# hsinnan75/MapCaller

Hardware: AMD Instinct MI355X
Metric: reads/sec (150 bp PE vs GRCh38) at 1/2/4/8 MI355X; SAM CIGAR bit-exact (higher is better)
Workload: dtype u64/int32; 1 GPU; synthetic GRCh38-sized genome, 3100 Mbp (synthetic: GRCh38 is unavailable offline; repeat landscape in the detail record), 4000000 pairs x 150 bp PE per step per GPU (sub 0.005, ins 0.001, del 0.001 per base), -alg ksw2

## Files before the change

mapcaller_amd/csrc/mcx_pack.h:

```cpp
#ifndef MCX_PACK_H
#define MCX_PACK_H
#include "mcx_fm.h"

namespace mcx {

static inline MCX_HD uint32_t pack_alignbyte(uint32_t hi, uint32_t lo, unsigned b)
{
#if defined(__HIP_DEVICE_COMPILE__)
    return __builtin_amdgcn_alignbyte(hi, lo, b);
#else
    return (uint32_t)((((uint64_t)hi << 32) | lo) >> (8 * (b & 3)));
#endif
}

static inline MCX_HD U4 load16_span(const U4 *base16, uint64_t A, int n)
{
    const U4 *q = base16 + (A >> 4);
    const U4 lo = q[0];
    const unsigned sh = (unsigned)(A & 15);
    if (sh == 0) return lo;
    U4 hi; hi.x = hi.y = hi.z = hi.w = 0;
    if ((int)sh + n > 16) hi = q[1];
    const unsigned qd = sh >> 2, b = sh & 3;
    uint32_t s0, s1, s2, s3, s4;
    switch (qd) {
    case 0: s0 = lo.x; s1 = lo.y; s2 = lo.z; s3 = lo.w; s4 = hi.x; break;
    case 1: s0 = lo.y; s1 = lo.z; s2 = lo.w; s3 = hi.x; s4 = hi.y; break;
    case 2: s0 = lo.z; s1 = lo.w; s2 = hi.x; s3 = hi.y; s4 = hi.z; break;
    default: s0 = lo.w; s1 = hi.x; s2 = hi.y; s3 = hi.z; s4 = hi.w; break;
    }
    U4 r;
    r.x = pack_alignbyte(s1, s0, b); r.y = pack_alignbyte(s2, s1, b);
    r.z = pack_alignbyte(s3, s2, b); r.w = pack_alignbyte(s4, s3, b);
    return r;
}

static inline MCX_HD void pack4(uint32_t w, bool comp, uint32_t &codes, uint32_t &flags, uint32_t &lower)
{
    const uint32_t c = w & 0xDFDFDFDFu;
#define MCX_ZERO_BYTES(t) (~((((t) & 0x7F7F7F7Fu) + 0x7F7F7F7Fu) | (t) | 0x7F7F7F7Fu))
    const uint32_t member = (MCX_ZERO_BYTES(c ^ 0x41414141u) | MCX_ZERO_BYTES(c ^ 0x43434343u) | MCX_ZERO_BYTES(c ^ 0x47474747u) | MCX_ZERO_BYTES(c ^ 0x54545454u)) >> 7;
#undef MCX_ZERO_BYTES
    const uint32_t h = (c >> 1) & 0x03030303u;
    uint32_t code = h ^ ((h >> 1) & 0x01010101u);
    if (comp) code ^= 0x03030303u;
    code &= member * 3u;
    const uint32_t y = __builtin_bswap32(code), n = __builtin_bswap32(member ^ 0x01010101u);
    codes = (y | (y >> 6) | (y >> 12) | (y >> 18)) & 0xFFu;
    flags = (n | (n >> 7) | (n >> 14) | (n >> 21)) & 0xFu;
    const uint32_t l = __builtin_bswap32((w >> 5) & 0x01010101u);
    lower = (l | (l >> 7) | (l >> 14) | (l >> 21)) & 0xFu;
}

static inline MCX_HD void pack16_span(const U4 *base16, uint64_t A0, int rlen, int flipped, int i0, uint32_t &codes, uint32_t &flags, uint32_t &odd)
{
    int n = rlen - i0; if (n > 16) n = 16;
    codes = 0; flags = 0xFFFFu; odd = 0;
    if (n <= 0) return;
    const int a0 = flipped ? rlen - i0 - n : i0;
    U4 v = load16_span(base16, A0 + (uint64_t)a0, n);
    if (flipped) {
        const U4 t = v;
        v.x = __builtin_bswap32(t.w); v.y = __builtin_bswap32(t.z); v.z = __builtin_bswap32(t.y); v.w = __builtin_bswap32(t.x);
    }
    uint32_t c0, f0, c1, f1, c2, f2, c3, f3, l0, l1, l2, l3;
    pack4(v.x, flipped != 0, c0, f0, l0); pack4(v.y, flipped != 0, c1, f1, l1); pack4(v.z, flipped != 0, c2, f2, l2); pack4(v.w, flipped != 0, c3, f3, l3);
    uint32_t c = (c0 << 24) | (c1 << 16) | (c2 << 8) | c3, f = (f0 << 12) | (f1 << 8) | (f2 << 4) | f3, o = f | (l0 << 12) | (l1 << 8) | (l2 << 4) | l3;
    if (n < 16) {
        const int pad = 16 - n;
        if (flipped) { c <<= 2 * pad; f = (f << pad) & 0xFFFFu; o = (o << pad) & 0xFFFFu; }
        else { c &= ~0u << (2 * pad); o &= ~0u << pad; }
        f |= (1u << pad) - 1u;
        if (!flipped) f &= 0xFFFFu;
    }
    codes = c; flags = f; odd = o & 0xFFFFu;
}

static inline MCX_HD void pack_row_ends(int rlen, uint32_t *row)
{
    const int nc = (rlen + 15) >> 4, nmw = (rlen + 31) >> 5;
    row[nc] = 0u;
    row[nc + 1 + nmw] = 0xFFFFFFFFu;
}

static inline MCX_HD void pack_unit32(const U4 *base16, uint64_t A0, int rlen, int flipped, int m, uint32_t *row, uint32_t &has_n, uint32_t &odd)
{
    const int nc = (rlen + 15) >> 4;
    uint32_t c0, f0, c1, f1, o0, o1;
    pack16_span(base16, A0, rlen, flipped, 32 * m, c0, f0, o0);
    pack16_span(base16, A0, rlen, flipped, 32 * m + 16, c1, f1, o1);
    row[2 * m] = c0;
    if (2 * m + 1 < nc) row[2 * m + 1] = c1;
    row[nc + 1 + m] = (f0 << 16) | f1;
    const int left = rlen - 32 * m;
    has_n = ((f0 << 16) | f1) & (left >= 32 ? ~0u : ~(0xFFFFFFFFu >> left));
    odd = o0 | o1;
}

}
#endif
```

mapcaller_amd/csrc/mcx_pipeline.hip:

```cpp
#include "mcx_ctx.h"
#include "mcx_pack.h"
#include <hipcub/hipcub.hpp>

static thread_local std::string g_err;
static int fail(int code, const std::string &msg) { g_err = msg; return code; }
int mcx_set_error(int code, const std::string &msg) { return fail(code, msg); }
extern "C" const char *mcx_last_error(void) { return g_err.c_str(); }
extern "C" int mcx_device_count(void)
{
    int n = 0;
    if (hipGetDeviceCount(&n) != hipSuccess) return 0;
    return n;
}

struct EndsLds { int64_t pos[kLdsEnds]; int32_t chr[kLdsEnds]; };

static __device__ __forceinline__ void stage_ends(IndexView &ix, EndsLds &l)
{
    if (ix.n_ends <= kLdsEnds) {
        for (int i = threadIdx.x; i < ix.n_ends; i += blockDim.x) { l.pos[i] = ix.end_pos[i]; l.chr[i] = ix.end_chr[i]; }
        __syncthreads();
        ix.end_pos = l.pos; ix.end_chr = l.chr;
    }
}

static __device__ __forceinline__ void make_reads(const Ctx &cx, const ReadBatch &rb, uint32_t pair, ReadRef rd[2])
{
    const int nr = cx.pm.paired ? 2 : 1;
    for (int s = 0; s < nr; s++) {
        uint32_t r = pair * nr + s;
        rd[s].ascii = rb.bases + rb.off[r];
        rd[s].rlen = (int32_t)(rb.off[r + 1] - rb.off[r]);
        rd[s].flipped = (cx.pm.paired && s == 1) ? 1 : 0;
        rd[s].codes = (cx.packed && !(cx.read_ext[r] >> 31)) ? cx.packed + (uint64_t)r * cx.wpad : nullptr;
#ifdef MCX_DEBUG_NO_CODES
        rd[s].codes = nullptr;
#endif
    }
}

struct SeedOut {
    uint2 *tasks;
    uint32_t *n_tasks;
    uint32_t task_cap;
    uint32_t *read_ext;
    uint32_t *read_blocks;
    const uint32_t *packed;
    int wpad;
    uint32_t *queue;
    const uint8_t *src_state; Layout src_lay; Caps src_caps;
};

static __device__ __forceinline__ void pack_read_part(const ReadBatch &rb, uint32_t r, int m, int paired, int wpad, uint32_t *out, uint32_t *any_n, uint8_t *odd_flag)
{
    const uint32_t a = rb.off[r];
    const int rlen = (int)(rb.off[r + 1] - a), flipped = (paired && (r & 1)) ? 1 : 0, nmw = (rlen + 31) >> 5;
    if (packed_words(rlen) > wpad) return;
    uint32_t *o = out + (uint64_t)r * wpad;
    const uint8_t *p = rb.bases + a;
    const uint32_t sh = (uint32_t)((uintptr_t)p & 15);
    if (m < nmw) {
        uint32_t has_n, odd;
        pack_unit32((const U4 *)(p - sh), (uint64_t)sh, rlen, flipped, m, o, has_n, odd);
        if (odd_flag && odd) atomicOr((uint32_t *)(odd_flag + (r & ~3u)), 2u << (8 * (r & 3)));
        if (has_n) atomicOr(any_n, 1u);
    } else if (m == nmw) pack_row_ends(rlen, o);
}

__global__ void __launch_bounds__(256) k_pack_reads(ReadBatch rb, int paired, int wpad, int tpr, uint32_t *out, uint32_t *any_n, uint8_t *odd_flag)
{
    const uint64_t t = (uint64_t)blockIdx.x * blockDim.x + threadIdx.x;
    const uint32_t r = (uint32_t)(t / (uint32_t)tpr);
    if (r < rb.n_reads) pack_read_part(rb, r, (int)(t % (uint32_t)tpr), paired, wpad, out, any_n, odd_flag);
}

void pack_reads(const ReadBatch &rb, int paired, int wpad, int tpr, uint32_t *out, uint32_t *any_n, uint8_t *odd_flag, hipStream_t s)
{
    k_pack_reads<<<(unsigned)(((uint64_t)rb.n_reads * (uint64_t)tpr + 255) / 256), 256, 0, s>>>(rb, paired, wpad, tpr, out, any_n, odd_flag);
}

constexpr int kSeedReadsPerLane = 4;


static inline int seed_reads_per_lane(uint64_t n_reads) { return n_reads >= (uint64_t)1 << 21 ? kSeedReadsPerLane : (n_reads >= (uint64_t)1 << 19 ? 2 : 1); }

#ifndef MCX_SEED_WAVES
#define MCX_SEED_WAVES 1
#endif
#ifdef MCX_SEED_STATS
__device__ unsigned long long g_seed_hist[2][24];
#endif
__global__ void __launch_bounds__(256, MCX_SEED_WAVES) k_seed(Ctx cx, ReadBatch rb, PairSel sel, SeedOut so, int pk_words, int reads_per_lane, int fm_budget)
{
    extern __shared__ uint32_t pk_lds[];
    const int nr = cx.pm.paired ? 2 : 1;
    const uint32_t total = sel.n * nr;
    const int lane = threadIdx.x & 63;
    const uint64_t lt_mask = lane == 0 ? 0ull : (~0ull >> (64 - lane));
    const uint32_t chunk = 64u * (uint32_t)reads_per_lane;
    PackedRead pk; pk.w = pk_lds + threadIdx.x; pk.stride = blockDim.x; pk.n_code = 0;
    bool have = false;
    uint32_t lr = 0, r = 0, nm = 0;
    int rlen = 0, p = 0, n = 0;
    int64_t ext = 0, blocks = 0;
    Hit *hits = nullptr;
    uint32_t has_n = 0;
    int cap = cx.caps.hit_seed;
    auto finish_read = [&]() {
        so.read_ext[r] = (uint32_t)ext | (has_n << 31); so.read_blocks[r] = (uint32_t)blocks | ((uint32_t)n << 20);
#ifdef MCX_SEED_STATS
        { const int bk = blocks ? 64 - __clzll((unsigned long long)blocks) : 0; atomicAdd(&g_seed_hist[0][bk], 1ull); atomicAdd(&g_seed_hist[1][bk], (unsigned long long)blocks); }
#endif
        if (cx.ix.sa_full) return;
        const int keep = n <= cx.caps.hit_seed ? n : 0;
        int todo = 0;
        for (int i = 0; i < keep; i++) if (!(hits[i].len & kHitResolved)) todo++;
        uint32_t at = todo ? atomicAdd(so.n_tasks, (uint32_t)todo) : 0u;
        for (int i = 0; i < keep; i++) {
            if (hits[i].len & kHitResolved) { hits[i].len &= ~kHitResolved; continue; }
            if (at < so.task_cap) so.tasks[at] = make_uint2(lr, (uint32_t)i);
            at++;
        }
    };
    SeedWalk walk; walk.phase = 0;
    uint32_t q_next = 0, q_end = 0;
    bool dry = false;
    for (;;) {
        const uint64_t need = __ballot(!have);
        bool fresh = false;
        if (need && !dry) {
            const uint32_t rank = (uint32_t)__popcll(need & lt_mask), want = (uint32_t)__popcll(need);
            uint32_t given = 0;
            while (given < want) {
                if (q_next == q_end) {
                    uint32_t b = 0;
                    if (lane == 0) b = atomicAdd(so.queue, chunk);
                    b = __shfl(b, 0, 64);
                    if (b >= total) { dry = true; break; }
                    q_next = b; q_end = min(b + chunk, total);
                }
                const uint32_t take = min(want - given, q_end - q_next);
                if (!have && !fresh && rank >= given && rank < given + take) { lr = q_next + (rank - given); fresh = true; }
                q_next += take; given += take;
            }
        }
        if (fresh) {
            r = sel_pair(sel, lr / nr) * nr + lr % nr;
            rlen = (int)(rb.off[r + 1] - rb.off[r]);
            hits = pair_state(cx.state, cx.lay, cx.caps, lr / nr).hits[lr % nr];
            n = 0; p = 0; ext = 0; blocks = 0; has_n = 0; walk.phase = 0;
            const int words = packed_words(rlen);
            if (so.src_state && !((so.read_ext[r] | (nr == 2 ? so.read_ext[r ^ 1u] : 0u)) >> 31)) {
                const PairState src = pair_state((uint8_t *)so.src_state, so.src_lay, so.src_caps, r / nr);
                const int m = src.hdr->n_hits[r % nr], n0 = (int)(so.read_blocks[r] >> 20);
                for (int i = 0; i < m; i++) hits[i] = src.hits[r % nr][i];
                Hit none; none.gPos = 0; none.rPos = 0; none.len = 0;
                for (int i = m; i < n0; i++) hits[i] = none;
                fresh = false;
            } else
            if (rlen > 0 && words <= pk_words) {
                const U4 *src = (const U4 *)(so.packed + (uint64_t)r * so.wpad);
                for (int k = 0; k < words; k += 4) {
                    const U4 v = src[k >> 2];
                    pk.w[k * pk.stride] = v.x;
                    if (k + 1 < words) pk.w[(k + 1) * pk.stride] = v.y;
                    if (k + 2 < words) pk.w[(k + 2) * pk.stride] = v.z;
                    if (k + 3 < words) pk.w[(k + 3) * pk.stride] = v.w;
                }
                pk.n_code = ((rlen + 15) >> 4) + 1;
                {
                    const int nmw = (rlen + 31) >> 5;
                    uint32_t any = 0;
                    for (int m = 0; m < nmw; m++) {
                        uint32_t w = pk.w[(pk.n_code + m) * pk.stride];
                        if (m == nmw - 1 && (rlen & 31)) w &= ~(0xFFFFFFFFu >> (rlen & 31));
                        any |= w;
                    }
                    has_n = any ? 1u : 0u;
                }
                have = seed_next_start(pk, rlen, p, nm);
            }
            if (!have && fresh) finish_read();
        }
        if (!__ballot(have)) { if (dry) break; continue; }
        if (have && walk.phase == 0) seed_begin(cx.ix, pk, rlen, nm, p, walk);
        if (have && walk.phase == 1) seed_fm(cx.ix, pk, rlen, p, walk, blocks, fm_budget);
        if (have && walk.phase == 2) seed_compare_wide(cx.ix, pk, rlen, p, walk, 1 << 30);
        if (have && walk.phase == 3) {
            seed_take(cx.ix, p, walk, hits, cap, n, ext);
            if (!seed_next_start(pk, rlen, p, nm)) { finish_read(); have = false; }
        }
    }
}

__global__ void __launch_bounds__(256) k_sa(Ctx cx, SeedOut so, int paired, uint32_t *lf_total)
{
    const uint32_t n = min(*so.n_tasks, so.task_cap);
    const int nr = paired ? 2 : 1;
    for (uint32_t t = blockIdx.x * blockDim.x + threadIdx.x; t < n; t += gridDim.x * blockDim.x) {
        const uint2 task = so.tasks[t];
        PairState st = pair_state(cx.state, cx.lay, cx.caps, task.x / nr);
        Hit &h = st.hits[task.x % nr][task.y];
        int lf = 0;
        h.gPos = (int64_t)fm_sa(cx.ix, (uint64_t)h.gPos, lf);
        if (lf_total && lf) atomicAdd(lf_total, (uint32_t)lf);
    }
}

struct RescueList { uint32_t *ids; uint32_t *n; uint32_t cap; };
struct EarlyList { uint32_t *ids; int32_t *est; uint32_t *n; uint32_t cap; uint32_t *n_hits; };

constexpr int kWorkClasses = 6;
static __device__ __forceinline__ int work_class(uint32_t hits) { return hits > 64 ? 0 : hits > 32 ? 1 : hits > 16 ? 2 : hits > 8 ? 3 : hits > 4 ? 4 : 5; }

static __device__ __forceinline__ int pair_work_class(const PairSel &sel, uint32_t local, const uint32_t *read_blocks, int nr, const uint8_t *done = nullptr)
{
    if (done && done[local]) return -1;
    const uint32_t pair = sel_pair(sel, local);
    return work_class((read_blocks[pair * nr] >> 20) + (nr == 2 ? read_blocks[pair * nr + 1] >> 20 : 0u));
}

constexpr int kOrderTile = 16;

__global__ void __launch_bounds__(256) k_order_count(PairSel sel, const uint32_t *read_blocks, int nr, uint32_t *counts, const uint8_t *done)
{
    __shared__ uint32_t n_cls[kWorkClasses];
    if (threadIdx.x < kWorkClasses) n_cls[threadIdx.x] = 0u;
    __syncthreads();
    const uint32_t base = blockIdx.x * (256u * kOrderTile);
    for (int t = 0; t < kOrderTile; t++) {
        const uint32_t local = base + t * 256u + threadIdx.x;
        const int cls = local < sel.n ? pair_work_class(sel, local, read_blocks, nr, done) : -1;
#pragma unroll
        for (int k = 0; k < kWorkClasses; k++) {
            const uint64_t m = __ballot(cls == k);
            if ((threadIdx.x & 63) == 0 && m) atomicAdd(&n_cls[k], (uint32_t)__popcll(m));
        }
    }
    __syncthreads();
    if (threadIdx.x < kWorkClasses && n_cls[threadIdx.x]) atomicAdd(counts + threadIdx.x * kCntPad, n_cls[threadIdx.x]);
}

__global__ void __launch_bounds__(256) k_order_place(PairSel sel, const uint32_t *read_blocks, int nr, uint32_t *counts, uint32_t *order, const uint8_t *done)
{
    __shared__ uint32_t n_cls[kWorkClasses], at_cls[kWorkClasses];
    if (threadIdx.x < kWorkClasses) n_cls[threadIdx.x] = 0u;
    __syncthreads();
    const uint32_t base = blockIdx.x * (256u * kOrderTile);
    const int lane = threadIdx.x & 63;
    int cls[kOrderTile];
#pragma unroll
    for (int t = 0; t < kOrderTile; t++) {
        const uint32_t local = base + t * 256u + threadIdx.x;
        cls[t] = local < sel.n ? pair_work_class(sel, local, read_blocks, nr, done) : -1;
#pragma unroll
        for (int k = 0; k < kWorkClasses; k++) {
            const uint64_t m = __ballot(cls[t] == k);
            if (lane == 0 && m) atomicAdd(&n_cls[k], (uint32_t)__popcll(m));
        }
    }
    __syncthreads();
    if (threadIdx.x < kWorkClasses) {
        uint32_t first = 0;
        for (int k = 0; k < (int)threadIdx.x; k++) first += counts[k * kCntPad];
        const uint32_t mine = n_cls[threadIdx.x];
        at_cls[threadIdx.x] = first + (mine ? atomicAdd(counts + (8 + threadIdx.x) * kCntPad, mine) : 0u);
    }
    __syncthreads();
#pragma unroll
    for (int t = 0; t < kOrderTile; t++) {
        const uint32_t local = base + t * 256u + threadIdx.x;
#pragma unroll
        for (int k = 0; k < kWorkClasses; k++) {
            const uint64_t m = __ballot(cls[t] == k);
            uint32_t b = 0;
            if (lane == 0 && m) b = atomicAdd(&at_cls[k], (uint32_t)__popcll(m));
            b = __shfl(b, 0, 64);
            if (cls[t] == k) order[b + (uint32_t)__popcll(m & ((1ull << lane) - 1ull))] = local;
        }
    }
}

struct SimpleLater {
    uint32_t *pairs;
    SimpleJob *jobs;
    SimpleRes *res;
    uint32_t *job_list;
    uint32_t *n_pairs, *n_jobs;
    uint32_t cap;
};

template <bool NW, int MODE, bool DETAIL>
__global__ void __launch_bounds__(256) k_simple(Ctx cx, ReadBatch rb, uint32_t n_pairs, const int32_t *est, const uint32_t *read_blocks, AlnRec *recs, PairOut *pout,
                                                uint8_t *done, uint32_t *pool_over, uint32_t *n_done, SimpleLater sl)
{
    __shared__ EndsLds ends;
    __shared__ uint16_t cig_stage[256 * 2 * kSimpleRuns];
    __shared__ uint32_t job_stage[MODE == kDpCollect ? 3 * kSimpleJobs * 256 : 1];
    stage_ends(cx.ix, ends);
    const uint32_t slot = blockIdx.x * blockDim.x + threadIdx.x;
    const int nr = cx.pm.paired ? 2 : 1;
    uint16_t *stage = cig_stage + threadIdx.x;
    const uint32_t n_slots = MODE == kDpReplay ? min(*sl.n_pairs, sl.cap) : n_pairs;
    bool ok = slot < n_slots;
    const uint32_t pair = MODE == kDpReplay ? (ok ? sl.pairs[slot] : 0u) : slot;
    SimpleRead sr[2];
    int rl[2] = {0, 0};
    typename std::conditional<DETAIL, SimpleDetail, SimpleNoDetail>::type det;
    SimpleDpIo io;
    io.mode = MODE == kDpCollect && !sl.pairs ? kDpNone : MODE;
    io.jobs = MODE == kDpCollect ? job_stage + threadIdx.x : nullptr; io.job_stride = 256;
    io.res = MODE == kDpReplay ? sl.res + (uint64_t)slot * kSimpleJobs : nullptr;
    io.n = 0; io.read = 0;
    bool later = false;
    if (ok) {
        const PairState st = pair_state(cx.state, cx.lay, cx.caps, pair);
#pragma unroll
        for (int s = 0; s < 2; s++) {
            if (s < nr && ok) {
                const uint32_t r = pair * nr + s;
                const int nh = (int)(read_blocks[r] >> 20);
                rl[s] = (int)(rb.off[r + 1] - rb.off[r]);
                io.read = r;
                ok = nh >= 1 && nh <= kSimpleHits && !(cx.read_ext[r] >> 31);
                if (ok) {
                    if constexpr (DETAIL) { uint8_t *rec = cx.detail + (uint64_t)r * cx.dlay.stride; det.frags = (Frag *)(rec + sizeof(DetailHdr)); det.ops = rec + cx.dlay.off_ops; }
                    const int how = simple_read<NW, uint16_t>(cx.ix, cx.pm, rl[s], cx.packed + (uint64_t)r * cx.wpad, st.hits[s], nh, sr[s], stage + s * kSimpleRuns * 256, 256, io, det);
                    ok = how != kSimpleNo;
                    later = later || how == kSimpleLater;
                }
            }
        }
        if (ok && nr == 2) ok = simple_pair_ok(sr[0], sr[1], est[pair]);
    }
    if (MODE == kDpCollect) {
        const bool wait = ok && later;
        const uint32_t at = wave_reserve(sl.n_pairs, wait ? 1u : 0u);
        const bool kept = wait && at < sl.cap;
        const uint32_t jat = wave_reserve(sl.n_jobs, kept ? (uint32_t)io.n : 0u);
        if (kept) {
            sl.pairs[at] = pair;
            for (int k = 0; k < io.n; k++) {
                const uint32_t *w = job_stage + (3 * k) * 256 + threadIdx.x;
                sl.jobs[(uint64_t)at * kSimpleJobs + k] = simple_job_unpack(w[0], w[256], w[512], pair * (uint32_t)nr, nr);
                sl.job_list[jat + k] = at * kSimpleJobs + (uint32_t)k;
            }
            done[pair] = 2;
        }
        if (wait) ok = false;
        later = kept;
    }
    const uint32_t want = ok ? (uint32_t)sr[0].n_cig + (nr == 2 ? (uint32_t)sr[1].n_cig : 0u) : 0u;
    const uint32_t at = wave_reserve(cx.cig_pool_n, want);
    const uint64_t took = __ballot(ok);
    if ((threadIdx.x & 63) == 0 && took) atomicAdd(n_done, (uint32_t)__popcll(took));
    if (slot >= n_slots) return;
    if (ok && at + want > cx.cig_pool_cap) { atomicOr(pool_over, 1u); ok = false; }
    if (!later) done[pair] = ok ? 1 : 0;
    if (!ok) return;
    const uint32_t off[2] = {at, at + (uint32_t)sr[0].n_cig};
#pragma unroll
    for (int s = 0; s < 2; s++) {
        if (s >= nr) break;
        for (int k = 0; k < sr[s].n_cig; k++) cx.cig_pool[off[s] + k] = (uint32_t)stage[(s * kSimpleRuns + k) * 256];
    }
    AlnRec rec2[2];
    PairOut po;
    simple_pair(cx, nr == 2, sr[0], sr[nr - 1], rl[0], rl[nr - 1], est[pair], rec2, off, po);
    recs[(uint64_t)pair * nr] = rec2[0];
    if (nr == 2) recs[(uint64_t)pair * nr + 1] = rec2[1];
    pout[pair] = po;
    if constexpr (DETAIL) {
#pragma unroll
        for (int s = 0; s < 2; s++) {
            if (s >= nr) break;
            const DetailHdr d = simple_detail_hdr(cx.ix, nr == 2, s, sr[0], sr[nr - 1]);
            *(DetailHdr *)(cx.detail + ((uint64_t)pair * nr + s) * cx.dlay.stride) = d;
        }
    }
}

// ... 2335 lines not shown
```

Before: 549.2 million reads/s.

## Streamline read packing with perm-based base coding and 2D launch

Base-to-2-bit encoding now uses a byte-permute lookup in place of the per-byte zero-detect cascade. Reads of 16 or more bases load 16 unaligned bytes directly rather than stitching aligned vectors. The odd-flag work is specialised away by a template when it is not needed, and the row-end write is folded into the last working thread, which drops one thread per read. A 2D workgroup removes the per-thread integer division. The aim is fewer ALU operations and threads in the pack kernel, but it adds template variants and relies on unaligned 16-byte loads staying within the read buffer.

```diff
diff --git a/mapcaller_amd/csrc/mcx_pack.h b/mapcaller_amd/csrc/mcx_pack.h
--- a/mapcaller_amd/csrc/mcx_pack.h
+++ b/mapcaller_amd/csrc/mcx_pack.h
@@ -35,45 +35,80 @@
     return r;
 }
 
+static inline MCX_HD uint32_t pack_perm(uint32_t hi, uint32_t lo, uint32_t sel)
+{
+#if defined(__HIP_DEVICE_COMPILE__)
+    return __builtin_amdgcn_perm(hi, lo, sel);
+#else
+    const uint64_t v = ((uint64_t)hi << 32) | lo;
+    uint32_t r = 0;
+    for (int k = 0; k < 4; k++) r |= (uint32_t)((v >> (8 * ((sel >> (8 * k)) & 7u))) & 0xFFu) << (8 * k);
+    return r;
+#endif
+}
+
+static inline MCX_HD U4 load16_bytes(const uint8_t *p)
+{
+    U4 v;
+    __builtin_memcpy(&v, p, 16);
+    return v;
+}
+
+static inline MCX_HD uint32_t pack_keep(uint32_t v)
+{
+#if defined(__HIP_DEVICE_COMPILE__)
+    asm volatile("" : "+v"(v));
+#endif
+    return v;
+}
+
+template <bool kOdd>
 static inline MCX_HD void pack4(uint32_t w, bool comp, uint32_t &codes, uint32_t &flags, uint32_t &lower)
 {
-    const uint32_t c = w & 0xDFDFDFDFu;
-#define MCX_ZERO_BYTES(t) (~((((t) & 0x7F7F7F7Fu) + 0x7F7F7F7Fu) | (t) | 0x7F7F7F7Fu))
-    const uint32_t member = (MCX_ZERO_BYTES(c ^ 0x41414141u) | MCX_ZERO_BYTES(c ^ 0x43434343u) | MCX_ZERO_BYTES(c ^ 0x47474747u) | MCX_ZERO_BYTES(c ^ 0x54545454u)) >> 7;
-#undef MCX_ZERO_BYTES
-    const uint32_t h = (c >> 1) & 0x03030303u;
-    uint32_t code = h ^ ((h >> 1) & 0x01010101u);
-    if (comp) code ^= 0x03030303u;
-    code &= member * 3u;
-    const uint32_t y = __builtin_bswap32(code), n = __builtin_bswap32(member ^ 0x01010101u);
-    codes = (y | (y >> 6) | (y >> 12) | (y >> 18)) & 0xFFu;
-    flags = (n | (n >> 7) | (n >> 14) | (n >> 21)) & 0xFu;
-    const uint32_t l = __builtin_bswap32((w >> 5) & 0x01010101u);
-    lower = (l | (l >> 7) | (l >> 14) | (l >> 21)) & 0xFu;
+    const uint32_t c = w & 0xDFDFDFDFu, k = w & 0x07070707u;
+    const uint32_t x = c ^ pack_perm(0x47FFFF54u, 0x43FF41FFu, k);
+    const uint32_t n = ((((x & 0x7F7F7F7Fu) + 0x7F7F7F7Fu) | x) >> 7) & 0x01010101u;
+    const uint32_t code = pack_perm(comp ? 0x01000000u : 0x02000003u, comp ? 0x02000300u : 0x01000000u, k) & ~(n * 3u);
+    uint32_t y = pack_keep(code | (code << 10)); y |= y << 20;
+    uint32_t f = pack_keep(n | (n << 9)); f |= f << 18;
+    codes = y >> 24;
+    flags = f >> 24;
+    if (kOdd) {
+        const uint32_t b = (w >> 5) & 0x01010101u;
+        uint32_t l = pack_keep(b | (b << 9)); l |= l << 18;
+        lower = l >> 24;
+    } else lower = 0;
 }
 
+template <bool kOdd>
+static inline MCX_HD void pack16_vec(U4 v, int flipped, int pad, bool at_end, uint32_t &codes, uint32_t &flags, uint32_t &odd)
+{
+    if (flipped) {
+        const U4 t = v;
+        v.x = __builtin_bswap32(t.w); v.y = __builtin_bswap32(t.z); v.z = __builtin_bswap32(t.y); v.w = __builtin_bswap32(t.x);
+    }
+    uint32_t c0, f0, c1, f1, c2, f2, c3, f3, l0, l1, l2, l3;
+    pack4<kOdd>(v.x, flipped != 0, c0, f0, l0); pack4<kOdd>(v.y, flipped != 0, c1, f1, l1); pack4<kOdd>(v.z, flipped != 0, c2, f2, l2); pack4<kOdd>(v.w, flipped != 0, c3, f3, l3);
+    uint32_t c = (c0 << 24) | (c1 << 16) | (c2 << 8) | c3, f = (f0 << 12) | (f1 << 8) | (f2 << 4) | f3, o = kOdd ? f | (l0 << 12) | (l1 << 8) | (l2 << 4) | l3 : 0u;
+    if (at_end) { c <<= 2 * pad; f = ((f << pad) & 0xFFFFu) | ((1u << pad) - 1u); o = (o << pad) & 0xFFFFu; }
+    else { c &= ~0u << (2 * pad); o &= ~0u << pad; f = (f | ((1u << pad) - 1u)) & 0xFFFFu; }
+    codes = c; flags = f; odd = o & 0xFFFFu;
+}
+
+static inline MCX_HD int pack_span_at(int rlen, int flipped, int i0, int n)
+{
+    return flipped ? rlen - i0 - n : i0 - (16 - n);
+}
+
+template <bool kOdd = true>
 static inline MCX_HD void pack16_span(const U4 *base16, uint64_t A0, int rlen, int flipped, int i0, uint32_t &codes, uint32_t &flags, uint32_t &odd)
 {
     int n = rlen - i0; if (n > 16) n = 16;
     codes = 0; flags = 0xFFFFu; odd = 0;
     if (n <= 0) return;
-    const int a0 = flipped ? rlen - i0 - n : i0;
-    U4 v = load16_span(base16, A0 + (uint64_t)a0, n);
-    if (flipped) {
-        const U4 t = v;
-        v.x = __builtin_bswap32(t.w); v.y = __builtin_bswap32(t.z); v.z = __builtin_bswap32(t.y); v.w = __builtin_bswap32(t.x);
-    }
-    uint32_t c0, f0, c1, f1, c2, f2, c3, f3, l0, l1, l2, l3;
-    pack4(v.x, flipped != 0, c0, f0, l0); pack4(v.y, flipped != 0, c1, f1, l1); pack4(v.z, flipped != 0, c2, f2, l2); pack4(v.w, flipped != 0, c3, f3, l3);
-    uint32_t c = (c0 << 24) | (c1 << 16) | (c2 << 8) | c3, f = (f0 << 12) | (f1 << 8) | (f2 << 4) | f3, o = f | (l0 << 12) | (l1 << 8) | (l2 << 4) | l3;
-    if (n < 16) {
-        const int pad = 16 - n;
-        if (flipped) { c <<= 2 * pad; f = (f << pad) & 0xFFFFu; o = (o << pad) & 0xFFFFu; }
-        else { c &= ~0u << (2 * pad); o &= ~0u << pad; }
-        f |= (1u << pad) - 1u;
-        if (!flipped) f &= 0xFFFFu;
-    }
-    codes = c; flags = f; odd = o & 0xFFFFu;
+    if (rlen >= 16) pack16_vec<kOdd>(load16_bytes((const uint8_t *)base16 + A0 + (uint64_t)pack_span_at(rlen, flipped, i0, n)), flipped, 16 - n, true, codes, flags, odd);
+    else
+        pack16_vec<kOdd>(load16_span(base16, A0 + (uint64_t)(flipped ? rlen - i0 - n : i0), n), flipped, 16 - n, flipped != 0, codes, flags, odd);
 }
 
 static inline MCX_HD void pack_row_ends(int rlen, uint32_t *row)
@@ -83,12 +118,23 @@
     row[nc + 1 + nmw] = 0xFFFFFFFFu;
 }
 
+template <bool kOdd = true>
 static inline MCX_HD void pack_unit32(const U4 *base16, uint64_t A0, int rlen, int flipped, int m, uint32_t *row, uint32_t &has_n, uint32_t &odd)
 {
     const int nc = (rlen + 15) >> 4;
     uint32_t c0, f0, c1, f1, o0, o1;
-    pack16_span(base16, A0, rlen, flipped, 32 * m, c0, f0, o0);
-    pack16_span(base16, A0, rlen, flipped, 32 * m + 16, c1, f1, o1);
+    if (rlen >= 16) {
+        const uint8_t *p = (const uint8_t *)base16 + A0;
+        const int i0 = 32 * m, left1 = rlen - i0 - 16, n0 = left1 >= 0 ? 16 : rlen - i0, n1 = left1 > 16 ? 16 : left1;
+        const U4 v0 = load16_bytes(p + pack_span_at(rlen, flipped, i0, n0));
+        const U4 v1 = load16_bytes(p + (n1 > 0 ? pack_span_at(rlen, flipped, i0 + 16, n1) : pack_span_at(rlen, flipped, i0, n0)));
+        pack16_vec<kOdd>(v0, flipped, 16 - n0, true, c0, f0, o0);
+        pack16_vec<kOdd>(v1, flipped, n1 > 0 ? 16 - n1 : 0, true, c1, f1, o1);
+        if (n1 <= 0) { c1 = 0; f1 = 0xFFFFu; o1 = 0; }
+    } else {
+        pack16_span<kOdd>(base16, A0, rlen, flipped, 32 * m, c0, f0, o0);
+        pack16_span<kOdd>(base16, A0, rlen, flipped, 32 * m + 16, c1, f1, o1);
+    }
     row[2 * m] = c0;
     if (2 * m + 1 < nc) row[2 * m + 1] = c1;
     row[nc + 1 + m] = (f0 << 16) | f1;
diff --git a/mapcaller_amd/csrc/mcx_pipeline.hip b/mapcaller_amd/csrc/mcx_pipeline.hip
--- a/mapcaller_amd/csrc/mcx_pipeline.hip
+++ b/mapcaller_amd/csrc/mcx_pipeline.hip
@@ -51,32 +51,52 @@
     const uint8_t *src_state; Layout src_lay; Caps src_caps;
 };
 
+template <bool kOdd>
 static __device__ __forceinline__ void pack_read_part(const ReadBatch &rb, uint32_t r, int m, int paired, int wpad, uint32_t *out, uint32_t *any_n, uint8_t *odd_flag)
 {
-    const uint32_t a = rb.off[r];
-    const int rlen = (int)(rb.off[r + 1] - a), flipped = (paired && (r & 1)) ? 1 : 0, nmw = (rlen + 31) >> 5;
+    const uint32_t a = rb.off[r], e = rb.off[r + 1];
+    const int rlen = (int)(e - a), flipped = (paired && (r & 1)) ? 1 : 0, nmw = (rlen + 31) >> 5;
     if (packed_words(rlen) > wpad) return;
     uint32_t *o = out + (uint64_t)r * wpad;
+    if (m == (nmw > 0 ? nmw - 1 : 0)) pack_row_ends(rlen, o);
+    if (m >= nmw) return;
     const uint8_t *p = rb.bases + a;
     const uint32_t sh = (uint32_t)((uintptr_t)p & 15);
-    if (m < nmw) {
-        uint32_t has_n, odd;
-        pack_unit32((const U4 *)(p - sh), (uint64_t)sh, rlen, flipped, m, o, has_n, odd);
-        if (odd_flag && odd) atomicOr((uint32_t *)(odd_flag + (r & ~3u)), 2u << (8 * (r & 3)));
-        if (has_n) atomicOr(any_n, 1u);
-    } else if (m == nmw) pack_row_ends(rlen, o);
-}
-
-__global__ void __launch_bounds__(256) k_pack_reads(ReadBatch rb, int paired, int wpad, int tpr, uint32_t *out, uint32_t *any_n, uint8_t *odd_flag)
-{
-    const uint64_t t = (uint64_t)blockIdx.x * blockDim.x + threadIdx.x;
-    const uint32_t r = (uint32_t)(t / (uint32_t)tpr);
-    if (r < rb.n_reads) pack_read_part(rb, r, (int)(t % (uint32_t)tpr), paired, wpad, out, any_n, odd_flag);
+    uint32_t has_n, odd;
+    pack_unit32<kOdd>((const U4 *)(p - sh), (uint64_t)sh, rlen, flipped, m, o, has_n, odd);
+    if (kOdd && odd) atomicOr((uint32_t *)(odd_flag + (r & ~3u)), 2u << (8 * (r & 3)));
+    if (has_n) atomicOr(any_n, 1u);
+}
+
+template <bool kOdd, bool kFlat>
+__global__ void __launch_bounds__(256) k_pack_reads(ReadBatch rb, int paired, int wpad, int parts, uint32_t *out, uint32_t *any_n, uint8_t *odd_flag)
+{
+    uint32_t r; int m;
+    if (kFlat) {
+        const uint64_t t = (uint64_t)blockIdx.x * blockDim.x + threadIdx.x, q = t / (uint32_t)parts;
+        if (q >= rb.n_reads) return;
+        r = (uint32_t)q; m = (int)(t - q * (uint32_t)parts);
+    } else {
+        r = blockIdx.x * blockDim.y + threadIdx.y; m = (int)threadIdx.x;
+        if (r >= rb.n_reads) return;
+    }
+    pack_read_part<kOdd>(rb, r, m, paired, wpad, out, any_n, odd_flag);
 }
 
 void pack_reads(const ReadBatch &rb, int paired, int wpad, int tpr, uint32_t *out, uint32_t *any_n, uint8_t *odd_flag, hipStream_t s)
 {
-    k_pack_reads<<<(unsigned)(((uint64_t)rb.n_reads * (uint64_t)tpr + 255) / 256), 256, 0, s>>>(rb, paired, wpad, tpr, out, any_n, odd_flag);
+    const int parts = std::max(tpr - 1, 1);
+    const uint32_t rpb = parts <= 256 ? 256u / (uint32_t)parts : 0u;
+    const uint64_t n_wg = rpb ? ((uint64_t)rb.n_reads + rpb - 1) / rpb : 0;
+    if (rpb && n_wg <= 0x7FFFFFFFull && rb.n_reads <= 0xFFFFFFFFu - 256u) {
+        const dim3 wg((unsigned)parts, rpb);
+        if (odd_flag) k_pack_reads<true, false><<<(unsigned)n_wg, wg, 0, s>>>(rb, paired, wpad, parts, out, any_n, odd_flag);
+        else k_pack_reads<false, false><<<(unsigned)n_wg, wg, 0, s>>>(rb, paired, wpad, parts, out, any_n, odd_flag);
+    } else {
+        const unsigned n_flat = (unsigned)(((uint64_t)rb.n_reads * (uint64_t)parts + 255) / 256);
+        if (odd_flag) k_pack_reads<true, true><<<n_flat, 256, 0, s>>>(rb, paired, wpad, parts, out, any_n, odd_flag);
+        else k_pack_reads<false, true><<<n_flat, 256, 0, s>>>(rb, paired, wpad, parts, out, any_n, odd_flag);
+    }
 }
 
 constexpr int kSeedReadsPerLane = 4;
```

New measurement: 555.4 million reads/s, median of 6. +1.1%, better.
